# DerrickWang005/CRIS.pytorch

Measured on AMD Instinct MI355X. Metric: train-step samples/sec, CRIS-R50 416x416 bs=64; loss parity vs ref, higher is better.
Workload: dtype bf16; 1 GPU; CRIS-R50 bf16 training step (fwd+BCE+bwd+Adam), 416x416, per-GPU bs=8, 17-token text, synthetic RefCOCO-shape batch resident in HBM (BASELINE.json configs[1]); global_batch=8, parallelism=dp1, launch=graph, graph_captured=True, syncbn_exchange=none, grad_exchange=none

## Files before the change

cris/pytorch_amd/csrc/elementwise.hip:

```cpp
#include <cmath>
#include "common.h"
#include "../../../include/cris_hip.h"

__device__ __forceinline__ void ld8f(const float* p, float* f) {
    const float4 a = *reinterpret_cast<const float4*>(p);
    const float4 b = *reinterpret_cast<const float4*>(p + 4);
    f[0] = a.x; f[1] = a.y; f[2] = a.z; f[3] = a.w; f[4] = b.x; f[5] = b.y; f[6] = b.z; f[7] = b.w;
}
__device__ __forceinline__ void ld8bf(const bf16_t* p, float* f) { unpack8(*reinterpret_cast<const uint4*>(p), f); }
__device__ __forceinline__ void st8bf(bf16_t* p, const float* f) { *reinterpret_cast<uint4*>(p) = pack8(f); }

#define GRID_STRIDE(idx, total) \
    for (long idx = (long)blockIdx.x * blockDim.x + threadIdx.x; idx < (total); idx += (long)gridDim.x * blockDim.x)

__global__ void stem_im2col_kernel(const float* __restrict__ img, int Bn, int H, int W, int OH, int OW, bf16_t* __restrict__ out) {
    const long total = (long)Bn * OH * OW * 4;
    const bool small = total < (1L << 24);
    GRID_STRIDE(idx, total) {
        const cris_idx4 q = cris_split4(idx, 4, OW, OH, small);
        const int kc = q.cv, ow = q.x, oh = q.y, b = q.b;
        const long m = idx >> 2;
        float v[8];
#pragma unroll
        for (int j = 0; j < 8; ++j) {
            const int k = kc * 8 + j;
            float x = 0.f;
            if (k < 27) {
                const int ci = k / 9, t = k - ci * 9;
                const int kh = t / 3, kw = t - kh * 3;
                const int ih = oh * 2 + kh - 1, iw = ow * 2 + kw - 1;
                if ((unsigned)ih < (unsigned)H && (unsigned)iw < (unsigned)W) x = img[(((size_t)b * 3 + ci) * H + ih) * W + iw];
            }
            v[j] = x;
        }
        st8bf(out + m * 32 + kc * 8, v);
    }
}

extern "C" int cris_stem_im2col(const float* img, int Bn, int H, int W, cris_bf16* out, void* stream) {
    CRIS_CHECK_ARG(img && out && Bn > 0 && H > 0 && W > 0, "bad args");
    const int OH = (H + 2 - 3) / 2 + 1, OW = (W + 2 - 3) / 2 + 1;
    const long total = (long)Bn * OH * OW * 4;
    hipLaunchKernelGGL(stem_im2col_kernel, dim3(cris_grid_1d(total, 256)), dim3(256), 0, (hipStream_t)stream, img, Bn, H, W, OH, OW, out);
    CRIS_LAUNCH_CHECK();
    return 0;
}

__global__ void avgpool2_fwd_kernel(const bf16_t* __restrict__ x, int ldx, int xcoff, int Bn, int H, int W, int C,
                                    bf16_t* __restrict__ y, int ldy, int ycoff) {
    const int CV = C >> 3, OH = H >> 1, OW = W >> 1;
    const long total = (long)Bn * OH * OW * CV;
    const bool small = total < (1L << 24);
    GRID_STRIDE(idx, total) {
        const cris_idx4 q = cris_split4(idx, CV, OW, OH, small);
        const int cv = q.cv, ow = q.x, oh = q.y, b = q.b;
        const long mo = ((long)b * OH + oh) * OW + ow;
        float o[8] = {0, 0, 0, 0, 0, 0, 0, 0}, t[8];
#pragma unroll
        for (int dy = 0; dy < 2; ++dy)
#pragma unroll
            for (int dx = 0; dx < 2; ++dx) {
                ld8bf(x + (((size_t)b * H + oh * 2 + dy) * W + ow * 2 + dx) * ldx + xcoff + cv * 8, t);
#pragma unroll
                for (int j = 0; j < 8; ++j) o[j] += t[j];
            }
#pragma unroll
        for (int j = 0; j < 8; ++j) o[j] *= 0.25f;
        st8bf(y + (size_t)mo * ldy + ycoff + cv * 8, o);
    }
}

extern "C" int cris_avgpool2_fwd(const cris_bf16* x, int ldx, int xcoff, int Bn, int H, int W, int C, cris_bf16* y,
                                 int ldy, int ycoff, void* stream) {
    CRIS_CHECK_ARG(x && y && !(H & 1) && !(W & 1) && !(C & 7) && !(ldx & 7) && !(ldy & 7) && !(xcoff & 7) && !(ycoff & 7), "bad args");
    const long total = (long)Bn * (H / 2) * (W / 2) * (C / 8);
    hipLaunchKernelGGL(avgpool2_fwd_kernel, dim3(cris_grid_1d(total, 256)), dim3(256), 0, (hipStream_t)stream, x, ldx, xcoff,
                       Bn, H, W, C, y, ldy, ycoff);
    CRIS_LAUNCH_CHECK();
    return 0;
}

__global__ void avgpool2_bwd_kernel(const bf16_t* __restrict__ dy, int lddy, int dycoff, int Bn, int H, int W, int C,
                                    bf16_t* __restrict__ dx, int lddx, int dxcoff, int accum) {
    const int CV = C >> 3, OH = H >> 1, OW = W >> 1;
    const long total = (long)Bn * H * W * CV;
    const bool small = total < (1L << 24);
    GRID_STRIDE(idx, total) {
        const cris_idx4 q = cris_split4(idx, CV, W, H, small);
        const int cv = q.cv, w = q.x, h = q.y, b = q.b;
        const long m = ((long)b * H + h) * W + w;
        float g[8];
        ld8bf(dy + (((size_t)b * OH + (h >> 1)) * OW + (w >> 1)) * lddy + dycoff + cv * 8, g);
        bf16_t* d = dx + (size_t)m * lddx + dxcoff + cv * 8;
        float o[8];
        if (accum) ld8bf(d, o);
#pragma unroll
        for (int j = 0; j < 8; ++j) o[j] = (accum ? o[j] : 0.f) + 0.25f * g[j];
        st8bf(d, o);
    }
}

extern "C" int cris_avgpool2_bwd(const cris_bf16* dy, int lddy, int dycoff, int Bn, int H, int W, int C, cris_bf16* dx,
                                 int lddx, int dxcoff, int accum, void* stream) {
    CRIS_CHECK_ARG(dy && dx && !(H & 1) && !(W & 1) && !(C & 7) && !(lddx & 7) && !(lddy & 7) && !(dxcoff & 7) && !(dycoff & 7), "bad args");
    const long total = (long)Bn * H * W * (C / 8);
    hipLaunchKernelGGL(avgpool2_bwd_kernel, dim3(cris_grid_1d(total, 256)), dim3(256), 0, (hipStream_t)stream, dy, lddy, dycoff,
                       Bn, H, W, C, dx, lddx, dxcoff, accum);
    CRIS_LAUNCH_CHECK();
    return 0;
}

__device__ __forceinline__ void up2_src(int dst, int n_in, int& i0, int& i1, float& l1) {
    float s = (dst + 0.5f) * 0.5f - 0.5f;
    s = fmaxf(s, 0.f);
    i0 = (int)s;
    i1 = i0 < n_in - 1 ? i0 + 1 : i0;
    l1 = s - (float)i0;
}

__global__ void upsample2_fwd_kernel(const bf16_t* __restrict__ x, int ldx, int xcoff, int Bn, int H, int W, int C,
                                     bf16_t* __restrict__ y, int ldy, int ycoff) {
    const int CV = C >> 3, OH = H * 2, OW = W * 2;
    const long total = (long)Bn * OH * OW * CV;
    const bool small = total < (1L << 24);
    GRID_STRIDE(idx, total) {
        const cris_idx4 q = cris_split4(idx, CV, OW, OH, small);
        const int cv = q.cv, ow = q.x, oh = q.y, b = q.b;
        const long mo = ((long)b * OH + oh) * OW + ow;
        int y0, y1, x0, x1;
        float ly, lx;
        up2_src(oh, H, y0, y1, ly);
        up2_src(ow, W, x0, x1, lx);
        const bf16_t* base = x + (size_t)b * H * W * ldx + xcoff + cv * 8;
        float a[8], bb[8], c[8], d[8], o[8];
        ld8bf(base + ((size_t)y0 * W + x0) * ldx, a);
        ld8bf(base + ((size_t)y0 * W + x1) * ldx, bb);
        ld8bf(base + ((size_t)y1 * W + x0) * ldx, c);
        ld8bf(base + ((size_t)y1 * W + x1) * ldx, d);
        const float w00 = (1.f - ly) * (1.f - lx), w01 = (1.f - ly) * lx, w10 = ly * (1.f - lx), w11 = ly * lx;
#pragma unroll
        for (int j = 0; j < 8; ++j) o[j] = w00 * a[j] + w01 * bb[j] + w10 * c[j] + w11 * d[j];
        st8bf(y + (size_t)mo * ldy + ycoff + cv * 8, o);
    }
}

extern "C" int cris_upsample2_fwd(const cris_bf16* x, int ldx, int xcoff, int Bn, int H, int W, int C, cris_bf16* y,
                                  int ldy, int ycoff, void* stream) {
    CRIS_CHECK_ARG(x && y && !(C & 7) && !(ldx & 7) && !(ldy & 7) && !(xcoff & 7) && !(ycoff & 7), "bad args");
    const long total = (long)Bn * H * W * 4 * (C / 8);
    hipLaunchKernelGGL(upsample2_fwd_kernel, dim3(cris_grid_1d(total, 256)), dim3(256), 0, (hipStream_t)stream, x, ldx, xcoff,
                       Bn, H, W, C, y, ldy, ycoff);
    CRIS_LAUNCH_CHECK();
    return 0;
}

__global__ void upsample2_bwd_kernel(const bf16_t* __restrict__ dy, int lddy, int dycoff, int Bn, int H, int W, int C,
                                     bf16_t* __restrict__ dx, int lddx, int dxcoff, int accum) {
    const int CV = C >> 3, OH = H * 2, OW = W * 2;
    const long total = (long)Bn * H * W * CV;
    const bool small = total < (1L << 24);
    GRID_STRIDE(idx, total) {
        const cris_idx4 q = cris_split4(idx, CV, W, H, small);
        const int cv = q.cv, ix = q.x, iy = q.y, b = q.b;
        const long m = ((long)b * H + iy) * W + ix;
        float acc[8] = {0, 0, 0, 0, 0, 0, 0, 0};
        const bf16_t* base = dy + (size_t)b * OH * OW * lddy + dycoff + cv * 8;
        for (int oy = max(0, 2 * iy - 2); oy <= min(OH - 1, 2 * iy + 2); ++oy) {
            int y0, y1; float ly;
            up2_src(oy, H, y0, y1, ly);
            float wy = 0.f;
            if (y0 == iy) wy += 1.f - ly;
            if (y1 == iy) wy += ly;
            if (wy == 0.f) continue;
            for (int ox = max(0, 2 * ix - 2); ox <= min(OW - 1, 2 * ix + 2); ++ox) {
                int x0, x1; float lx;
                up2_src(ox, W, x0, x1, lx);
                float wx = 0.f;
                if (x0 == ix) wx += 1.f - lx;
                if (x1 == ix) wx += lx;
                if (wx == 0.f) continue;
                float g[8];
                ld8bf(base + ((size_t)oy * OW + ox) * lddy, g);
                const float w = wy * wx;
#pragma unroll
                for (int j = 0; j < 8; ++j) acc[j] += w * g[j];
            }
        }
        bf16_t* d = dx + (size_t)m * lddx + dxcoff + cv * 8;
        if (accum) {
            float o[8];
            ld8bf(d, o);
#pragma unroll
            for (int j = 0; j < 8; ++j) acc[j] += o[j];
        }
        st8bf(d, acc);
    }
}

extern "C" int cris_upsample2_bwd(const cris_bf16* dy, int lddy, int dycoff, int Bn, int H, int W, int C, cris_bf16* dx,
                                  int lddx, int dxcoff, int accum, void* stream) {
    CRIS_CHECK_ARG(dy && dx && !(C & 7) && !(lddx & 7) && !(lddy & 7) && !(dxcoff & 7) && !(dycoff & 7), "bad args");
    const long total = (long)Bn * H * W * (C / 8);
    hipLaunchKernelGGL(upsample2_bwd_kernel, dim3(cris_grid_1d(total, 256)), dim3(256), 0, (hipStream_t)stream, dy, lddy, dycoff,
                       Bn, H, W, C, dx, lddx, dxcoff, accum);
    CRIS_LAUNCH_CHECK();
    return 0;
}

__device__ __forceinline__ float linspace_m1_1(int i, int n) {
    if (n == 1) return -1.f;
    const float step = 2.f / (float)(n - 1);
    return i < n / 2 ? -1.f + step * (float)i : 1.f - step * (float)(n - 1 - i);
}

__global__ void fill_coords_kernel(bf16_t* x, int ldx, int coff, int nfill, int Bn, int H, int W) {
    const long total = (long)Bn * H * W;
    GRID_STRIDE(m, total) {
        const int w = (int)(m % W);
        const int h = (int)((m / W) % H);
        bf16_t* d = x + (size_t)m * ldx + coff;
        d[0] = f2bf(linspace_m1_1(w, W));
        d[1] = f2bf(linspace_m1_1(h, H));
        for (int j = 2; j < nfill; ++j) d[j] = 0;
    }
}

extern "C" int cris_fill_coords(cris_bf16* x, int ldx, int coff, int nfill, int Bn, int H, int W, void* stream) {
    CRIS_CHECK_ARG(x && nfill >= 2, "bad args");
    hipLaunchKernelGGL(fill_coords_kernel, dim3(cris_grid_1d((long)Bn * H * W, 256)), dim3(256), 0, (hipStream_t)stream, x, ldx,
                       coff, nfill, Bn, H, W);
    CRIS_LAUNCH_CHECK();
    return 0;
}

__global__ void gather_samples_kernel(const bf16_t* __restrict__ x, int ldx, int xcoff, const int32_t* __restrict__ index,
                                      int R, int CV, bf16_t* __restrict__ y, int ldy, int ycoff, int total) {
    for (int idx = blockIdx.x * blockDim.x + threadIdx.x; idx < total; idx += gridDim.x * blockDim.x) {
        const int cv = idx % CV;
        const int row = idx / CV;
        const int k = row / R;
        const int r = row - k * R;
        const long src = (long)index[k] * R + r;
        const uint4 v = *reinterpret_cast<const uint4*>(x + (size_t)src * ldx + xcoff + cv * 8);
        *reinterpret_cast<uint4*>(y + (size_t)row * ldy + ycoff + cv * 8) = v;
    }
}

extern "C" int cris_gather_samples_bf16(const cris_bf16* x, int ldx, int xcoff, const int32_t* index, int K,
                                        int rows_per_sample, int C, cris_bf16* y, int ldy, int ycoff, void* stream) {
    CRIS_CHECK_ARG(x && y && index && K > 0 && rows_per_sample > 0 && C > 0, "bad args");
    CRIS_CHECK_ARG(!(C & 7) && !(ldx & 7) && !(ldy & 7) && !(xcoff & 7) && !(ycoff & 7) && xcoff >= 0 && ycoff >= 0 &&
                   xcoff + C <= ldx && ycoff + C <= ldy, "channels, leading dimensions and offsets: multiples of 8, slice inside the row");
    CRIS_CHECK_ARG((long)K * rows_per_sample * ldy * 2 < (1L << 31), "output extent of 2 GiB or more");
    const int total = K * rows_per_sample * (C / 8);
    hipLaunchKernelGGL(gather_samples_kernel, dim3(cris_grid_1d(total, 256)), dim3(256), 0, (hipStream_t)stream, x, ldx, xcoff,
                       index, rows_per_sample, C / 8, y, ldy, ycoff, total);
    CRIS_LAUNCH_CHECK();
    return 0;
}

__global__ void add_bf16_kernel(const bf16_t* a, int lda, int acoff, const bf16_t* b, int ldb, int bcoff, bf16_t* y, int ldy,
                                int ycoff, int M, int C) {
    const int CV = C >> 3;
    const long total = (long)M * CV;
    GRID_STRIDE(idx, total) {
        const int cv = (int)(idx % CV);
        const long m = idx / CV;
        float u[8], v[8];
        ld8bf(a + (size_t)m * lda + acoff + cv * 8, u);
        if (b) {
            ld8bf(b + (size_t)m * ldb + bcoff + cv * 8, v);
#pragma unroll
            for (int j = 0; j < 8; ++j) u[j] += v[j];
        }
        st8bf(y + (size_t)m * ldy + ycoff + cv * 8, u);
    }
}

extern "C" int cris_add_bf16(const cris_bf16* a, int lda, int acoff, const cris_bf16* b, int ldb, int bcoff, cris_bf16* y,
                             int ldy, int ycoff, int M, int C, void* stream) {
    CRIS_CHECK_ARG(a && y && !(C & 7) && !(lda & 7) && !(ldy & 7) && !(acoff & 7) && !(ycoff & 7) && (!b || (!(ldb & 7) && !(bcoff & 7))), "bad args");
    hipLaunchKernelGGL(add_bf16_kernel, dim3(cris_grid_1d((long)M * (C / 8), 256)), dim3(256), 0, (hipStream_t)stream, a, lda,
                       acoff, b, ldb, bcoff, y, ldy, ycoff, M, C);
    CRIS_LAUNCH_CHECK();
    return 0;
}

__global__ void add_rowtable_kernel(const bf16_t* a, int lda, const float* table, int trows, bf16_t* y, int ldy, int M, int C) {
    const int CV = C >> 3;
    const long total = (long)M * CV;
    GRID_STRIDE(idx, total) {
        const int cv = (int)(idx % CV);
        const long m = idx / CV;
        float u[8], v[8];
        ld8bf(a + (size_t)m * lda + cv * 8, u);
        ld8f(table + (size_t)(m % trows) * C + cv * 8, v);
#pragma unroll
        for (int j = 0; j < 8; ++j) u[j] += v[j];
        st8bf(y + (size_t)m * ldy + cv * 8, u);
    }
}

extern "C" int cris_add_rowtable(const cris_bf16* a, int lda, const float* table, int trows, cris_bf16* y, int ldy, int M,
                                 int C, void* stream) {
    CRIS_CHECK_ARG(a && table && y && trows > 0 && !(C & 7) && !(lda & 7) && !(ldy & 7), "bad args");
    hipLaunchKernelGGL(add_rowtable_kernel, dim3(cris_grid_1d((long)M * (C / 8), 256)), dim3(256), 0, (hipStream_t)stream, a,
                       lda, table, trows, y, ldy, M, C);
    CRIS_LAUNCH_CHECK();
    return 0;
}

__global__ void cast_f32_bf16_kernel(const float* x, bf16_t* y, long n) {
    GRID_STRIDE(i, n) y[i] = f2bf(x[i]);
}
extern "C" int cris_cast_f32_bf16(const float* x, cris_bf16* y, long n, void* stream) {
    CRIS_CHECK_ARG(x && y && n > 0, "bad args");
    hipLaunchKernelGGL(cast_f32_bf16_kernel, dim3(cris_grid_1d(n, 256)), dim3(256), 0, (hipStream_t)stream, x, y, n);
    CRIS_LAUNCH_CHECK();
    return 0;
}
__global__ void cast_bf16_f32_kernel(const bf16_t* x, float* y, long n, int accum) {
    GRID_STRIDE(i, n) y[i] = (accum ? y[i] : 0.f) + bf2f(x[i]);
}
extern "C" int cris_cast_bf16_f32(const cris_bf16* x, float* y, long n, int accum, void* stream) {
    CRIS_CHECK_ARG(x && y && n > 0, "bad args");
    hipLaunchKernelGGL(cast_bf16_f32_kernel, dim3(cris_grid_1d(n, 256)), dim3(256), 0, (hipStream_t)stream, x, y, n, accum);
    CRIS_LAUNCH_CHECK();
    return 0;
}
__global__ void quickgelu_fwd_kernel(const bf16_t* x, bf16_t* y, long nvec) {
    GRID_STRIDE(i, nvec) {
        float v[8];
        ld8bf(x + i * 8, v);
#pragma unroll
        for (int j = 0; j < 8; ++j) v[j] = v[j] / (1.f + __expf(-1.702f * v[j]));
        st8bf(y + i * 8, v);
    }
}
extern "C" int cris_quickgelu_fwd(const cris_bf16* x, cris_bf16* y, long n, void* stream) {
    CRIS_CHECK_ARG(x && y && n > 0 && !(n & 7), "n must be a multiple of 8");
    hipLaunchKernelGGL(quickgelu_fwd_kernel, dim3(cris_grid_1d(n / 8, 256)), dim3(256), 0, (hipStream_t)stream, x, y, n / 8);
    CRIS_LAUNCH_CHECK();
    return 0;
}
__global__ void quickgelu_bwd_kernel(const bf16_t* x, const bf16_t* dy, bf16_t* dx, long nvec) {
    GRID_STRIDE(i, nvec) {
        float v[8], g[8];
        ld8bf(x + i * 8, v);
        ld8bf(dy + i * 8, g);
#pragma unroll
        for (int j = 0; j < 8; ++j) {
            const float s = 1.f / (1.f + __expf(-1.702f * v[j]));
            g[j] *= s * (1.f + 1.702f * v[j] * (1.f - s));
        }
        st8bf(dx + i * 8, g);
    }
}
extern "C" int cris_quickgelu_bwd(const cris_bf16* x, const cris_bf16* dy, cris_bf16* dx, long n, void* stream) {
    CRIS_CHECK_ARG(x && dy && dx && n > 0 && !(n & 7), "n must be a multiple of 8");
    hipLaunchKernelGGL(quickgelu_bwd_kernel, dim3(cris_grid_1d(n / 8, 256)), dim3(256), 0, (hipStream_t)stream, x, dy, dx, n / 8);
    CRIS_LAUNCH_CHECK();
    return 0;
}
__global__ void cast_drop_kernel(const float* x, bf16_t* y, long n, float scale, uint32_t thresh, uint32_t seed, uint32_t stream_id,
                                 const uint32_t* seed_dev) {
    const uint32_t key = cris_drop_key(seed + (seed_dev ? seed_dev[0] : 0u), stream_id);
    GRID_STRIDE(i, n) {
        float v = x[i];
        if (thresh) v = cris_keep(key, (uint32_t)i, thresh) ? v * scale : 0.f;
        y[i] = f2bf(v);
    }
}
extern "C" int cris_cast_f32_bf16_drop(const float* x, cris_bf16* y, long n, float drop_p, uint32_t drop_thresh, uint32_t seed,
                                       uint32_t stream_id, const uint32_t* seed_dev, void* stream) {
    CRIS_CHECK_ARG(x && y && n > 0 && n < (1L << 32), "bad args");
    const float scale = drop_thresh ? 1.f / (1.f - drop_p) : 1.f;
    hipLaunchKernelGGL(cast_drop_kernel, dim3(cris_grid_1d(n, 256)), dim3(256), 0, (hipStream_t)stream, x, y, n, scale, drop_thresh,
                       seed, stream_id, seed_dev);
    CRIS_LAUNCH_CHECK();
    return 0;
}
__global__ void step_advance_kernel(int* step, uint32_t* seed, int* exchange_gen) {
    const int s = step[0];
    seed[0] = (uint32_t)s * 7919u + 17u;
    step[0] = s + 1;
    if (exchange_gen) exchange_gen[0] += 1;
}
extern "C" int cris_step_advance(int32_t* step, uint32_t* seed, int32_t* exchange_gen, void* stream) {
    CRIS_CHECK_ARG(step && seed, "bad args");
    hipLaunchKernelGGL(step_advance_kernel, dim3(1), dim3(1), 0, (hipStream_t)stream, step, seed, exchange_gen);
    CRIS_LAUNCH_CHECK();
    return 0;
}
__global__ void step_advance_micro_kernel(int* step, uint32_t* seed, int* exchange_gen, int micro, int accum) {
    int s = step[0];
    if (micro == 0) step[0] = s + 1;
    else s -= 1;
    seed[0] = ((uint32_t)s * (uint32_t)accum + (uint32_t)micro) * 7919u + 17u;
    if (exchange_gen) exchange_gen[0] += 1;
}
extern "C" int cris_step_advance_micro(int32_t* step, uint32_t* seed, int32_t* exchange_gen, int micro, int accum, void* stream) {
    CRIS_CHECK_ARG(step && seed && accum >= 1 && micro >= 0 && micro < accum, "bad args (0 <= micro < accum)");
    hipLaunchKernelGGL(step_advance_micro_kernel, dim3(1), dim3(1), 0, (hipStream_t)stream, step, seed, exchange_gen, micro, accum);
    CRIS_LAUNCH_CHECK();
    return 0;
}
template <int MODE>
__global__ __launch_bounds__(256) void grad_accumulate_kernel(float4* __restrict__ dst, const float4* __restrict__ src, long nvec) {
    const long stride = (long)gridDim.x * 256;
    long i = (long)blockIdx.x * 256 + threadIdx.x;
    for (; i + stride < nvec; i += 2 * stride) {
        float4 s0 = src[i], s1 = src[i + stride];
        if (MODE == 1) {
            const float4 d0 = dst[i], d1 = dst[i + stride];
            s0.x = d0.x + s0.x; s0.y = d0.y + s0.y; s0.z = d0.z + s0.z; s0.w = d0.w + s0.w;
            s1.x = d1.x + s1.x; s1.y = d1.y + s1.y; s1.z = d1.z + s1.z; s1.w = d1.w + s1.w;
        }
        dst[i] = s0;
        dst[i + stride] = s1;
    }
    if (i < nvec) {
        float4 s0 = src[i];
        if (MODE == 1) {
            const float4 d0 = dst[i];
            s0.x = d0.x + s0.x; s0.y = d0.y + s0.y; s0.z = d0.z + s0.z; s0.w = d0.w + s0.w;
        }
        dst[i] = s0;
    }
}
static int cris_cu_count() {
    static int cached[64];
    int dev = 0;
    if (hipGetDevice(&dev) != hipSuccess || dev < 0 || dev >= 64) return 256;
    if (!cached[dev]) {
        int cus = 0;
        if (hipDeviceGetAttribute(&cus, hipDeviceAttributeMultiprocessorCount, dev) != hipSuccess || cus <= 0) cus = 256;
        cached[dev] = cus;
    }
    return cached[dev];
}
extern "C" int cris_grad_accumulate(float* dst, const float* src, long n, int mode, void* stream) {
    CRIS_CHECK_ARG(dst && src && n > 0 && !(n & 3), "n must be a positive multiple of 4");
    CRIS_CHECK_ARG(!(((uintptr_t)dst | (uintptr_t)src) & 15), "dst and src must be 16-byte aligned");
    CRIS_CHECK_ARG(mode == 0 || mode == 1, "mode must be 0 (dst = src) or 1 (dst += src)");
    CRIS_CHECK_ARG(dst + n <= src || src + n <= dst, "dst and src overlap");
    const long nvec = n >> 2;
    const int grid = cris_grid_1d(nvec, 512, 8 * cris_cu_count());
    if (mode == 0)
        hipLaunchKernelGGL(grad_accumulate_kernel<0>, dim3(grid), dim3(256), 0, (hipStream_t)stream, (float4*)dst, (const float4*)src, nvec);
    else
        hipLaunchKernelGGL(grad_accumulate_kernel<1>, dim3(grid), dim3(256), 0, (hipStream_t)stream, (float4*)dst, (const float4*)src, nvec);
    CRIS_LAUNCH_CHECK();
    return 0;
}
__global__ void axpy_f32_kernel(float* dst, const float* src, float alpha, long n) {
    GRID_STRIDE(i, n) dst[i] += alpha * src[i];
}
extern "C" int cris_axpy_f32(float* dst, const float* src, float alpha, long n, void* stream) {
    CRIS_CHECK_ARG(dst && src && n > 0, "bad args");
    hipLaunchKernelGGL(axpy_f32_kernel, dim3(cris_grid_1d(n, 256)), dim3(256), 0, (hipStream_t)stream, dst, src, alpha, n);
    CRIS_LAUNCH_CHECK();
    return 0;
}
__global__ void embed_fwd_kernel(const int64_t* tokens, const float* table, const float* pos, int Bn, int L, int D, float* out) {
    const int DV = D >> 2;
    const long total = (long)Bn * L * DV;
    GRID_STRIDE(idx, total) {
        const int dv = (int)(idx % DV);
        const long r = idx / DV;
        const int l = (int)(r % L);
        const int64_t tok = tokens[r];
        const float4 e = *reinterpret_cast<const float4*>(table + (size_t)tok * D + dv * 4);
        const float4 q = *reinterpret_cast<const float4*>(pos + (size_t)l * D + dv * 4);
        *reinterpret_cast<float4*>(out + (size_t)r * D + dv * 4) = make_float4(e.x + q.x, e.y + q.y, e.z + q.z, e.w + q.w);
    }
}
extern "C" int cris_embed_fwd(const int64_t* tokens, const float* table, const float* pos, int Bn, int L, int D, float* out,
                              void* stream) {
    CRIS_CHECK_ARG(tokens && table && pos && out && !(D & 3), "bad args");
    hipLaunchKernelGGL(embed_fwd_kernel, dim3(cris_grid_1d((long)Bn * L * (D / 4), 256)), dim3(256), 0, (hipStream_t)stream,
                       tokens, table, pos, Bn, L, D, out);
    CRIS_LAUNCH_CHECK();
    return 0;
}
__global__ void embed_bwd_kernel(const int64_t* tokens, const float* dx, int Bn, int L, int D, float* dtable, float* dpos,
                                 unsigned char* row_live) {
    const long total = (long)Bn * L * D;
    const int R = Bn * L;
    GRID_STRIDE(idx, total) {
        const int d = (int)(idx % D);
        const int r = (int)(idx / D);
        const int64_t tok = tokens[r];
        bool first = true;
        for (int q = 0; q < r; ++q) first = first && tokens[q] != tok;
        if (first) {
            float a = 0.f;
            for (int q = r; q < R; ++q)
                if (tokens[q] == tok) a += dx[(size_t)q * D + d];
            dtable[(size_t)tok * D + d] = a;
            if (row_live && d == 0) row_live[tok] = 1;
        }
        if (r < L) {
            float a = 0.f;
            for (int b = 0; b < Bn; ++b) a += dx[((size_t)b * L + r) * D + d];
            dpos[(size_t)r * D + d] = a;
// ... 812 lines not shown
```

cris/pytorch_amd/csrc/norm.hip:

```cpp
#include "common.h"
#include "../../../include/cris_hip.h"
#include "p2p_ll.h"
#include <string.h>

#define BN_WIDE_MIN 128
#define BN_MERGE_MIN 512
#define BN_MERGE_SLICES 64

template <int PL>
__device__ __forceinline__ float bn_lane_sum(float (*sh)[17], float v, int pl, int cl) {
    __syncthreads();
    sh[pl][cl] = v;
    __syncthreads();
    if (PL == 64) {
        float g = 0.f;
        if (pl < 8) {
#pragma unroll
            for (int j = 0; j < 8; ++j) g += sh[pl * 8 + j][cl];
        }
        __syncthreads();
        if (pl < 8) sh[pl][cl] = g;
        __syncthreads();
    }
    float t = sh[0][cl];
// ... 972 lines not shown
#pragma unroll
        for (int u = 0; u < U; ++u) {
            const int mu = m + u * step;
            if (mu >= M) break;
            float y[8], dz[8], z[8], g[8], o[8];
            unpack8(ry[u], y);
            unpack8(rdz[u], dz);
            if (MASK == 1) unpack8(rz[u], z);
#pragma unroll
            for (int j = 0; j < 8; ++j) {
                bool pos = true;
                if (MASK == 1) pos = z[j] > 0.f;
                if (MASK == 2) pos = (y[j] * sc[j] + sh[j]) > 0.f;
                g[j] = pos ? dz[j] : 0.f;
                const float xh = (y[j] - mean[j]) * inv[j];
                o[j] = sc[j] * (g[j] - a0[j] - xh * s1[j] * invc);
            }
            cris_st16(dyb + (size_t)mu * p.lddy, pack8(o));
            if (want2) {
                float y2[8];
                unpack8(ry2[u], y2);
#pragma unroll
                for (int j = 0; j < 8; ++j) {
                    const float xh2 = (y2[j] - mean2[j]) * inv2[j];
                    o[j] = sc2[j] * (g[j] - a0[j] - xh2 * s3[j] * invc);
                }
                cris_st16(dy2b + (size_t)mu * p.lddy2, pack8(o));
            }
            if (dib) {
                if (di_acc) {
                    float old[8];
                    unpack8(rold[u], old);
#pragma unroll
                    for (int j = 0; j < 8; ++j) g[j] += old[j];
                }
                cris_st16(dib + (size_t)mu * p.lddi, pack8(g));
            }
        }
    }
}

extern "C" int cris_bn_bwd_apply(const cris_bn_bwd_params* pp, void* stream) {
    const cris_bn_bwd_params& p = *pp;
    CRIS_CHECK_ARG(p.dz && p.y && p.mean && p.invstd && p.sums && p.scale && p.dy, "null operand");
    CRIS_CHECK_ARG((p.C & 7) == 0 && (p.lddy & 7) == 0 && (p.dy_coff & 7) == 0 && p.count > 0.f, "geometry");
    CRIS_CHECK_ARG(!(p.relu && !p.pool && p.y2 && !p.z), "relu over two branches takes its mask from the stored output z");
    const long total = (long)p.Bn * p.H * p.W * (p.C >> 3);
    static const int use_fast = cris_env_int("CRIS_BN_APPLY_FAST", 1);
    const int cvs = bn_cv_shift(p.C);
    const bool aligned = (p.ldy & 7) == 0 && (p.y_coff & 7) == 0 && (p.lddz & 7) == 0 && (p.dz_coff & 7) == 0 &&
                         (!p.y2 || ((p.ldy2 & 7) == 0 && (p.y2_coff & 7) == 0 && p.z && (!p.dy2 || ((p.lddy2 & 7) == 0 && (p.dy2_coff & 7) == 0)))) &&
                         (!p.dident || ((p.lddi & 7) == 0 && (p.di_coff & 7) == 0));
    if (use_fast && cvs >= 0 && !p.pool && !p.mul && aligned) {
        const int mask = !p.relu ? 0 : (p.y2 || p.z) ? 1 : 2;
        if (mask != 1 || ((p.ldz & 7) == 0 && (p.z_coff & 7) == 0)) {
            const int grid = bn_fast_grid(total, p.y2 ? 2 : 4);
            typedef void (*fn_t)(const cris_bn_bwd_params, int);
            static const fn_t tab[2][3] = {{bn_bwd_apply_fast_kernel<0, false>, bn_bwd_apply_fast_kernel<1, false>, bn_bwd_apply_fast_kernel<2, false>},
                                           {bn_bwd_apply_fast_kernel<0, true>, bn_bwd_apply_fast_kernel<1, true>, bn_bwd_apply_fast_kernel<2, true>}};
            hipLaunchKernelGGL(tab[p.y2 ? 1 : 0][mask], dim3(grid), dim3(256), 0, (hipStream_t)stream, p, cvs);
            CRIS_LAUNCH_CHECK();
            return 0;
        }
    }
    hipLaunchKernelGGL(bn_bwd_apply_kernel, dim3(cris_grid_1d(total, 256)), dim3(256), 0, (hipStream_t)stream, p);
    CRIS_LAUNCH_CHECK();
    return 0;
}

#define LN_MAXV 4

template <bool WANT_MASK, int V = LN_MAXV>
__device__ __forceinline__ void ln_load_row(const void* x, int x_f32, size_t rowoff, int C, int lane, int in_relu,
                                            uint32_t in_thresh, float in_scale, uint32_t in_key, uint32_t row,
                                            float (&v)[V][8], float (&mask_out)[V][8]) {
#pragma unroll
    for (int i = 0; i < V; ++i) {
        const int c0 = (lane + 64 * i) * 8;
        if (c0 < C) {
            if (x_f32) load8f(reinterpret_cast<const float*>(x) + rowoff + c0, v[i]);
            else load8bf(reinterpret_cast<const bf16_t*>(x) + rowoff + c0, v[i]);
#pragma unroll
            for (int j = 0; j < 8; ++j) {
                float m = 1.f;
                if (in_relu && !(v[i][j] > 0.f)) m = 0.f;
                if (in_thresh) m = cris_keep(in_key, row * (uint32_t)C + (uint32_t)(c0 + j), in_thresh) ? m * in_scale : 0.f;
                v[i][j] *= m;
                if (WANT_MASK) mask_out[i][j] = m;
            }
        } else {
#pragma unroll
            for (int j = 0; j < 8; ++j) {
                v[i][j] = 0.f;
                if (WANT_MASK) mask_out[i][j] = 0.f;
            }
        }
    }
}

__global__ __launch_bounds__(256) void ln_fwd_kernel(const cris_ln_fwd_params p) {
    const int lane = threadIdx.x & 63;
    const int wave_g = blockIdx.x * 4 + (threadIdx.x >> 6);
    const int nwaves = gridDim.x * 4;
    const uint32_t sdev = p.seed_dev ? p.seed_dev[0] : 0u;
    const uint32_t in_key = cris_drop_key(p.in_seed + sdev, p.in_stream);
    const uint32_t out_key = cris_drop_key(p.out_seed + sdev, p.out_stream);
    const float in_scale = p.in_thresh ? 1.f / (1.f - p.in_drop_p) : 1.f;
    const float out_scale = p.out_thresh ? 1.f / (1.f - p.out_drop_p) : 1.f;
    const float invC = 1.f / (float)p.C;
    for (int row = wave_g; row < p.rows; row += nwaves) {
        float v[LN_MAXV][8];
        ln_load_row<false>(p.x, p.x_f32, (size_t)row * p.ldx, p.C, lane, p.in_relu, p.in_thresh, in_scale, in_key, (uint32_t)row,
                           v, v);
        float s = 0.f;
#pragma unroll
        for (int i = 0; i < LN_MAXV; ++i)
#pragma unroll
            for (int j = 0; j < 8; ++j) s += v[i][j];
        const float mean = wave_sum(s) * invC;
        float q = 0.f;
#pragma unroll
        for (int i = 0; i < LN_MAXV; ++i) {
            const int c0 = (lane + 64 * i) * 8;
            if (c0 < p.C) {
#pragma unroll
                for (int j = 0; j < 8; ++j) {
                    const float d = v[i][j] - mean;
                    q += d * d;
                }
            }
        }
        const float rstd = rsqrtf(wave_sum(q) * invC + p.eps);
        if (lane == 0) {
            p.mean[row] = mean;
            p.rstd[row] = rstd;
        }
#pragma unroll
        for (int i = 0; i < LN_MAXV; ++i) {
            const int c0 = (lane + 64 * i) * 8;
            if (c0 >= p.C) continue;
            float ga[8], be[8], o[8];
            load8f(p.gamma + c0, ga);
            load8f(p.beta + c0, be);
#pragma unroll
            for (int j = 0; j < 8; ++j) o[j] = (v[i][j] - mean) * rstd * ga[j] + be[j];
            const size_t oo = (size_t)row * p.C + c0;
            if (p.y) cris_st16(p.y + oo, pack8(o));
            if (p.ypos) {
                float pe[8], t[8];
                load8f(p.pos + (size_t)(row % p.pos_rows) * p.C + c0, pe);
#pragma unroll
                for (int j = 0; j < 8; ++j) t[j] = o[j] + pe[j];
                cris_st16(p.ypos + oo, pack8(t));
            }
            if (p.out_f32) {
                float r[8];
                if (p.resid) load8f(p.resid + oo, r);
                else {
#pragma unroll
                    for (int j = 0; j < 8; ++j) r[j] = 0.f;
                }
#pragma unroll
                for (int j = 0; j < 8; ++j) {
                    float t = o[j];
                    if (p.out_thresh) t = cris_keep(out_key, (uint32_t)row * (uint32_t)p.C + (uint32_t)(c0 + j), p.out_thresh) ? t * out_scale : 0.f;
                    r[j] += t;
                }
                *reinterpret_cast<float4*>(p.out_f32 + oo) = make_float4(r[0], r[1], r[2], r[3]);
                *reinterpret_cast<float4*>(p.out_f32 + oo + 4) = make_float4(r[4], r[5], r[6], r[7]);
            }
        }
    }
}

extern "C" int cris_ln_fwd(const cris_ln_fwd_params* pp, void* stream) {
    const cris_ln_fwd_params& p = *pp;
    CRIS_CHECK_ARG(p.x && p.gamma && p.beta && p.mean && p.rstd && p.rows > 0, "null operand");
    CRIS_CHECK_ARG((p.C & 7) == 0 && p.C <= 64 * 8 * LN_MAXV && (p.ldx & 7) == 0, "C must be a multiple of 8, <= 2048");
    CRIS_CHECK_ARG(!p.ypos || (p.pos && p.pos_rows > 0), "ypos needs pos");
    CRIS_CHECK_ARG((long)p.rows * p.C < (1L << 32), "dropout index overflow");
    const int grid = cris_grid_1d(p.rows, 4, 2048);
    hipLaunchKernelGGL(ln_fwd_kernel, dim3(grid), dim3(256), 0, (hipStream_t)stream, p);
    CRIS_LAUNCH_CHECK();
    return 0;
}

template <int V>
__global__ __launch_bounds__(256) void ln_bwd_kernel(const cris_ln_bwd_params p) {
    __shared__ float sg[2][64 * 8 * V];
    const int lane = threadIdx.x & 63;
    const int wave_g = blockIdx.x * 4 + (threadIdx.x >> 6);
    const int nwaves = gridDim.x * 4;
    for (int i = threadIdx.x; i < 2 * 64 * 8 * V; i += 256) (&sg[0][0])[i] = 0.f;
    __syncthreads();
    const uint32_t sdev = p.seed_dev ? p.seed_dev[0] : 0u;
    const uint32_t in_key = cris_drop_key(p.in_seed + sdev, p.in_stream);
    const uint32_t out_key = cris_drop_key(p.out_seed + sdev, p.out_stream);
    const float in_scale = p.in_thresh ? 1.f / (1.f - p.in_drop_p) : 1.f;
    const float out_scale = p.out_thresh ? 1.f / (1.f - p.out_drop_p) : 1.f;
    const float invC = 1.f / (float)p.C;
    float dga[V][8], dbe[V][8];
#pragma unroll
    for (int i = 0; i < V; ++i)
#pragma unroll
        for (int j = 0; j < 8; ++j) dga[i][j] = dbe[i][j] = 0.f;

    for (int row = wave_g; row < p.rows; row += nwaves) {
        float v[V][8], msk[V][8];
        ln_load_row<true, V>(p.x, p.x_f32, (size_t)row * p.ldx, p.C, lane, p.in_relu, p.in_thresh, in_scale, in_key, (uint32_t)row,
                          v, msk);
        const float mean = p.mean[row], rstd = p.rstd[row];
        float a[V][8];
        float s1 = 0.f, s2 = 0.f;
#pragma unroll
        for (int i = 0; i < V; ++i) {
            const int c0 = (lane + 64 * i) * 8;
            if (c0 < p.C) {
                const size_t oo = (size_t)row * p.C + c0;
                float g[8], t[8], ga[8];
#pragma unroll
                for (int j = 0; j < 8; ++j) g[j] = 0.f;
                if (p.dy) {
                    load8bf(p.dy + oo, t);
#pragma unroll
                    for (int j = 0; j < 8; ++j) g[j] += t[j];
                }
                if (p.dypos) {
                    load8bf(p.dypos + oo, t);
#pragma unroll
                    for (int j = 0; j < 8; ++j) g[j] += t[j];
                }
                if (p.dout_f32) {
                    load8f(p.dout_f32 + oo, t);
#pragma unroll
                    for (int j = 0; j < 8; ++j) {
                        float d = t[j];
                        if (p.out_thresh) d = cris_keep(out_key, (uint32_t)row * (uint32_t)p.C + (uint32_t)(c0 + j), p.out_thresh) ? d * out_scale : 0.f;
                        g[j] += d;
                    }
                }
                load8f(p.gamma + c0, ga);
#pragma unroll
                for (int j = 0; j < 8; ++j) {
                    const float xh = (v[i][j] - mean) * rstd;
                    v[i][j] = xh;
                    dga[i][j] += g[j] * xh;
                    dbe[i][j] += g[j];
                    a[i][j] = g[j] * ga[j];
                    s1 += a[i][j];
                    s2 += a[i][j] * xh;
                }
            } else {
#pragma unroll
                for (int j = 0; j < 8; ++j) a[i][j] = 0.f;
            }
        }
        const float m1 = wave_sum(s1) * invC, m2 = wave_sum(s2) * invC;
#pragma unroll
        for (int i = 0; i < V; ++i) {
            const int c0 = (lane + 64 * i) * 8;
            if (c0 >= p.C) continue;
            float o[8];
#pragma unroll
            for (int j = 0; j < 8; ++j) o[j] = rstd * (a[i][j] - m1 - v[i][j] * m2) * msk[i][j];
            const size_t xo = (size_t)row * p.ldx + c0;
            if (p.dx_f32) {
                float* d = reinterpret_cast<float*>(p.dx) + xo;
                if (p.dx_accum) {
                    float old[8];
                    load8f(d, old);
#pragma unroll
                    for (int j = 0; j < 8; ++j) o[j] += old[j];
                }
                *reinterpret_cast<float4*>(d) = make_float4(o[0], o[1], o[2], o[3]);
                *reinterpret_cast<float4*>(d + 4) = make_float4(o[4], o[5], o[6], o[7]);
            } else {
                cris_st16(reinterpret_cast<bf16_t*>(p.dx) + xo, pack8(o));
            }
        }
    }
    for (int w = 0; w < 4; ++w) {
        if ((int)(threadIdx.x >> 6) == w) {
#pragma unroll
            for (int i = 0; i < V; ++i) {
                const int c0 = (lane + 64 * i) * 8;
                if (c0 < p.C) {
#pragma unroll
                    for (int j = 0; j < 8; ++j) {
                        sg[0][c0 + j] += dga[i][j];
                        sg[1][c0 + j] += dbe[i][j];
                    }
                }
            }
        }
        __syncthreads();
    }
    float* part = p.part + (size_t)blockIdx.x * 2 * p.C;
    for (int c = threadIdx.x; c < p.C; c += 256) {
        part[c] = sg[0][c];
        part[p.C + c] = sg[1][c];
    }
}

static int ln_bwd_grid(int rows) {
    static const int max_grid = cris_env_int("CRIS_LN_BWD_BLOCKS", 512);
    return cris_grid_1d(rows, 4, max_grid);
}
extern "C" int cris_ln_bwd_parts(int rows) { return ln_bwd_grid(rows); }

extern "C" int cris_ln_bwd(const cris_ln_bwd_params* pp, void* stream) {
    const cris_ln_bwd_params& p = *pp;
    CRIS_CHECK_ARG(p.x && p.gamma && p.mean && p.rstd && p.dx && p.part && p.rows > 0, "null operand");
    CRIS_CHECK_ARG(p.dy || p.dypos || p.dout_f32, "no incoming gradient");
    CRIS_CHECK_ARG((p.C & 7) == 0 && p.C <= 64 * 8 * LN_MAXV && (p.ldx & 7) == 0, "C must be a multiple of 8, <= 2048");
    CRIS_CHECK_ARG(!p.dx_accum || p.dx_f32, "accumulate only into fp32");
    static const int narrow = cris_env_int("CRIS_LN_BWD_V", 1);
    const dim3 grid(ln_bwd_grid(p.rows));
    if (narrow && p.C <= 512) hipLaunchKernelGGL(ln_bwd_kernel<1>, grid, dim3(256), 0, (hipStream_t)stream, p);
    else if (narrow && p.C <= 1024) hipLaunchKernelGGL(ln_bwd_kernel<2>, grid, dim3(256), 0, (hipStream_t)stream, p);
    else hipLaunchKernelGGL(ln_bwd_kernel<LN_MAXV>, grid, dim3(256), 0, (hipStream_t)stream, p);
    CRIS_LAUNCH_CHECK();
    return 0;
}

__global__ __launch_bounds__(256) void sum_group_kernel(const cris_sum_group g) {
    __shared__ float sh[4][64];
    int ei = 0;
#pragma unroll
    for (int i = 1; i < CRIS_SUM_GROUP_MAX; ++i) ei += g.block_start[i] <= (int)blockIdx.x ? 1 : 0;
    const cris_sum_entry e = g.e[ei];
    const int cl = threadIdx.x & 63, pl = threadIdx.x >> 6;
    const int c = (blockIdx.x - g.block_start[ei]) * 64 + cl;
    float a = 0.f;
    if (c < e.ncol)
        for (int i = pl; i < e.nparts; i += 4) a += e.part[(size_t)i * e.ld + c];
    sh[pl][cl] = a;
    __syncthreads();
    if (pl == 0 && c < e.ncol) e.out[c] = (sh[0][cl] + sh[1][cl]) + (sh[2][cl] + sh[3][cl]);
}

extern "C" int cris_sum_tables(const cris_sum_group* gp, void* stream) {
    CRIS_CHECK_ARG(gp && gp->n > 0 && gp->n <= CRIS_SUM_GROUP_MAX, "1 .. CRIS_SUM_GROUP_MAX tables per launch");
    cris_sum_group g = *gp;
    int start = 0;
    for (int i = 0; i < g.n; ++i) {
        CRIS_CHECK_ARG(g.e[i].part && g.e[i].out && g.e[i].nparts > 0 && g.e[i].ncol > 0 && g.e[i].ld >= g.e[i].ncol, "bad table");
        g.block_start[i] = start;
        start += cris_cdiv(g.e[i].ncol, 64);
    }
    for (int i = g.n; i <= CRIS_SUM_GROUP_MAX; ++i) g.block_start[i] = start;
    hipLaunchKernelGGL(sum_group_kernel, dim3(start), dim3(256), 0, (hipStream_t)stream, g);
    CRIS_LAUNCH_CHECK();
    return 0;
}
```

Measured before the change: 671.3 samples/s.

## Add quad-output upsample2 fwd, gather bwd, lean wide LN bwd, prefetching sum_tables

Adds an upsample2 forward kernel in which each thread loads a 3x3 input neighbourhood once and writes four output pixels, replacing four separate threads that each reloaded four neighbours. It also adds a backward kernel that enumerates exactly the four output rows and columns touching each input pixel, with fixed bilinear weights. A new LayerNorm backward kernel for C>1024 prefetches the next row's x and dy into registers and recomputes masks from bits to save registers. The partial-table sum kernel batches 16 independent loads per thread to expose memory-level parallelism. All four paths are on by default behind env flags. The code trades extra register pressure and a hardcoded half-pixel weight pattern for fewer redundant loads.

```diff
diff --git a/cris/pytorch_amd/csrc/elementwise.hip b/cris/pytorch_amd/csrc/elementwise.hip
--- a/cris/pytorch_amd/csrc/elementwise.hip
+++ b/cris/pytorch_amd/csrc/elementwise.hip
@@ -144,9 +144,62 @@
     }
 }
 
+__device__ __forceinline__ void up2_blend(const uint4 ra, const uint4 rb, const uint4 rc, const uint4 rd, float ly, float lx, bf16_t* dst) {
+    float a[8], bb[8], c[8], d[8], o[8];
+    unpack8(ra, a);
+    unpack8(rb, bb);
+    unpack8(rc, c);
+    unpack8(rd, d);
+    const float w00 = (1.f - ly) * (1.f - lx), w01 = (1.f - ly) * lx, w10 = ly * (1.f - lx), w11 = ly * lx;
+#pragma unroll
+    for (int j = 0; j < 8; ++j) o[j] = w00 * a[j] + w01 * bb[j] + w10 * c[j] + w11 * d[j];
+    st8bf(dst, o);
+}
+__device__ __forceinline__ uint4 up2_sel(bool first, const uint4 a, const uint4 b) {
+    return make_uint4(first ? a.x : b.x, first ? a.y : b.y, first ? a.z : b.z, first ? a.w : b.w);
+}
+
+__global__ void upsample2_fwd_quad_kernel(const bf16_t* __restrict__ x, int ldx, int xcoff, int Bn, int H, int W, int C,
+                                          bf16_t* __restrict__ y, int ldy, int ycoff) {
+    const int CV = C >> 3, OW = W * 2;
+    const long total = (long)Bn * H * W * CV;
+    const bool small = total < (1L << 24);
+    GRID_STRIDE(idx, total) {
+        const cris_idx4 q = cris_split4(idx, CV, W, H, small);
+        const int cv = q.cv, ix = q.x, iy = q.y, b = q.b;
+        int r[3], c[3], y1e, x1e;
+        float lye, lyo, lxe, lxo;
+        up2_src(2 * iy, H, r[0], y1e, lye);
+        up2_src(2 * iy + 1, H, r[1], r[2], lyo);
+        up2_src(2 * ix, W, c[0], x1e, lxe);
+        up2_src(2 * ix + 1, W, c[1], c[2], lxo);
+        const bf16_t* base = x + (size_t)b * H * W * ldx + xcoff + cv * 8;
+        uint4 v[3][3];
+#pragma unroll
+        for (int a = 0; a < 3; ++a)
+#pragma unroll
+            for (int e = 0; e < 3; ++e) v[a][e] = *reinterpret_cast<const uint4*>(base + ((size_t)r[a] * W + c[e]) * ldx);
+        const bool ym = y1e == r[1], xm = x1e == c[1];
+        uint4 t[3];
+#pragma unroll
+        for (int e = 0; e < 3; ++e) t[e] = up2_sel(ym, v[1][e], v[2][e]);
+        bf16_t* d = y + (((size_t)b * 2 * H + 2 * iy) * OW + 2 * ix) * ldy + ycoff + cv * 8;
+        up2_blend(v[0][0], up2_sel(xm, v[0][1], v[0][2]), t[0], up2_sel(xm, t[1], t[2]), lye, lxe, d);
+        up2_blend(v[0][1], v[0][2], t[1], t[2], lye, lxo, d + ldy);
+        up2_blend(v[1][0], up2_sel(xm, v[1][1], v[1][2]), v[2][0], up2_sel(xm, v[2][1], v[2][2]), lyo, lxe, d + (size_t)OW * ldy);
+        up2_blend(v[1][1], v[1][2], v[2][1], v[2][2], lyo, lxo, d + (size_t)OW * ldy + ldy);
+    }
+}
+
 extern "C" int cris_upsample2_fwd(const cris_bf16* x, int ldx, int xcoff, int Bn, int H, int W, int C, cris_bf16* y,
                                   int ldy, int ycoff, void* stream) {
     CRIS_CHECK_ARG(x && y && !(C & 7) && !(ldx & 7) && !(ldy & 7) && !(xcoff & 7) && !(ycoff & 7), "bad args");
+    if (cris_env_int("CRIS_UPSAMPLE2_QUAD", 1)) {
+        hipLaunchKernelGGL(upsample2_fwd_quad_kernel, dim3(cris_grid_1d((long)Bn * H * W * (C / 8), 256)), dim3(256), 0, (hipStream_t)stream,
+                           x, ldx, xcoff, Bn, H, W, C, y, ldy, ycoff);
+        CRIS_LAUNCH_CHECK();
+        return 0;
+    }
     const long total = (long)Bn * H * W * 4 * (C / 8);
     hipLaunchKernelGGL(upsample2_fwd_kernel, dim3(cris_grid_1d(total, 256)), dim3(256), 0, (hipStream_t)stream, x, ldx, xcoff,
                        Bn, H, W, C, y, ldy, ycoff);
@@ -197,10 +250,69 @@
     }
 }
 
+__device__ __forceinline__ void up2_hits(int i, int n, int on, int (&o)[4], float (&w)[4], bool (&ok)[4]) {
+    o[0] = max(2 * i - 1, 0);      w[0] = 0.25f;                      ok[0] = i >= 1;
+    o[1] = 2 * i;                  w[1] = i >= 1 ? 0.75f : 1.f;       ok[1] = true;
+    o[2] = 2 * i + 1;              w[2] = i == n - 1 ? 1.f : 0.75f;   ok[2] = true;
+    o[3] = min(2 * i + 2, on - 1); w[3] = 0.25f;                      ok[3] = i < n - 1;
+}
+
+__global__ void upsample2_bwd_enum_kernel(const bf16_t* __restrict__ dy, int lddy, int dycoff, int Bn, int H, int W, int C,
+                                          bf16_t* __restrict__ dx, int lddx, int dxcoff, int accum) {
+    const int CV = C >> 3, OH = H * 2, OW = W * 2;
+    const long total = (long)Bn * H * W * CV;
+    const bool small = total < (1L << 24);
+    GRID_STRIDE(idx, total) {
+        const cris_idx4 q = cris_split4(idx, CV, W, H, small);
+        const int cv = q.cv, ix = q.x, iy = q.y, b = q.b;
+        const long m = ((long)b * H + iy) * W + ix;
+        int oy[4], ox[4];
+        float wy[4], wx[4];
+        bool oky[4], okx[4];
+        up2_hits(iy, H, OH, oy, wy, oky);
+        up2_hits(ix, W, OW, ox, wx, okx);
+        const bf16_t* base = dy + (size_t)b * OH * OW * lddy + dycoff + cv * 8;
+        uint4 r[4][4];
+#pragma unroll
+        for (int a = 0; a < 4; ++a)
+#pragma unroll
+            for (int e = 0; e < 4; ++e) r[a][e] = *reinterpret_cast<const uint4*>(base + ((size_t)oy[a] * OW + ox[e]) * lddy);
+        bf16_t* d = dx + (size_t)m * lddx + dxcoff + cv * 8;
+        uint4 old = make_uint4(0, 0, 0, 0);
+        if (accum) old = *reinterpret_cast<const uint4*>(d);
+        float acc[8] = {0, 0, 0, 0, 0, 0, 0, 0};
+#pragma unroll
+        for (int a = 0; a < 4; ++a)
+#pragma unroll
+            for (int e = 0; e < 4; ++e) {
+                if (oky[a] && okx[e]) {
+                    float g[8];
+                    unpack8(r[a][e], g);
+                    const float w = wy[a] * wx[e];
+#pragma unroll
+                    for (int j = 0; j < 8; ++j) acc[j] += w * g[j];
+                }
+            }
+        if (accum) {
+            float o[8];
+            unpack8(old, o);
+#pragma unroll
+            for (int j = 0; j < 8; ++j) acc[j] += o[j];
+        }
+        st8bf(d, acc);
+    }
+}
+
 extern "C" int cris_upsample2_bwd(const cris_bf16* dy, int lddy, int dycoff, int Bn, int H, int W, int C, cris_bf16* dx,
                                   int lddx, int dxcoff, int accum, void* stream) {
     CRIS_CHECK_ARG(dy && dx && !(C & 7) && !(lddx & 7) && !(lddy & 7) && !(dxcoff & 7) && !(dycoff & 7), "bad args");
     const long total = (long)Bn * H * W * (C / 8);
+    if (cris_env_int("CRIS_UPSAMPLE2_QUAD", 1)) {
+        hipLaunchKernelGGL(upsample2_bwd_enum_kernel, dim3(cris_grid_1d(total, 256)), dim3(256), 0, (hipStream_t)stream, dy, lddy, dycoff,
+                           Bn, H, W, C, dx, lddx, dxcoff, accum);
+        CRIS_LAUNCH_CHECK();
+        return 0;
+    }
     hipLaunchKernelGGL(upsample2_bwd_kernel, dim3(cris_grid_1d(total, 256)), dim3(256), 0, (hipStream_t)stream, dy, lddy, dycoff,
                        Bn, H, W, C, dx, lddx, dxcoff, accum);
     CRIS_LAUNCH_CHECK();
diff --git a/cris/pytorch_amd/csrc/norm.hip b/cris/pytorch_amd/csrc/norm.hip
--- a/cris/pytorch_amd/csrc/norm.hip
+++ b/cris/pytorch_amd/csrc/norm.hip
@@ -1298,6 +1298,179 @@
     }
 }
 
+__device__ __forceinline__ uint32_t ln_lean_xh(const uint4 xr, int in_relu, uint32_t in_thresh, float in_scale, uint32_t in_key,
+                                               uint32_t idx0, float mean, float rstd, float* xh) {
+#pragma clang fp contract(off)
+    float v[8];
+    unpack8(xr, v);
+    uint32_t bits = 0;
+#pragma unroll
+    for (int j = 0; j < 8; ++j) {
+        float m = 1.f;
+        if (in_relu && !(v[j] > 0.f)) m = 0.f;
+        if (in_thresh) m = cris_keep(in_key, idx0 + (uint32_t)j, in_thresh) ? m * in_scale : 0.f;
+        v[j] *= m;
+        bits |= m != 0.f ? 1u << j : 0u;
+        xh[j] = (v[j] - mean) * rstd;
+    }
+    return bits;
+}
+__device__ __forceinline__ void ln_lean_xh_again(const uint4 xr, uint32_t bits, float mval, float mean, float rstd, float* xh, float* msk) {
+#pragma clang fp contract(off)
+    float v[8];
+    unpack8(xr, v);
+#pragma unroll
+    for (int j = 0; j < 8; ++j) {
+        const float m = (bits >> j) & 1u ? mval : 0.f;
+        v[j] *= m;
+        msk[j] = m;
+        xh[j] = (v[j] - mean) * rstd;
+    }
+}
+
+__device__ __forceinline__ void ln_lean_load(const cris_ln_bwd_params& p, const bf16_t* xb, int row, int lane, uint4 (&xr)[LN_MAXV],
+                                             uint4 (&dyr)[LN_MAXV], float& mean, float& rstd) {
+    const bf16_t* dyb = p.dy ? p.dy : xb;
+    const size_t xo = (size_t)row * p.ldx, dyo = p.dy ? (size_t)row * p.C : xo;
+#pragma unroll
+    for (int i = 0; i < LN_MAXV; ++i) {
+        const int c0 = (lane + 64 * i) * 8, cc = c0 < p.C ? c0 : 0;
+        xr[i] = *reinterpret_cast<const uint4*>(xb + xo + cc);
+        dyr[i] = *reinterpret_cast<const uint4*>(dyb + dyo + cc);
+    }
+    mean = p.mean[row];
+    rstd = p.rstd[row];
+}
+
+__global__ __launch_bounds__(256) void ln_bwd_lean_kernel(const cris_ln_bwd_params p) {
+    constexpr int V = LN_MAXV;
+    __shared__ float sg[2][64 * 8 * V];
+    __shared__ float sgam[64 * 8 * V];
+    const int lane = threadIdx.x & 63;
+    const int wave_g = blockIdx.x * 4 + (threadIdx.x >> 6);
+    const int nwaves = gridDim.x * 4;
+    for (int i = threadIdx.x; i < 2 * 64 * 8 * V; i += 256) (&sg[0][0])[i] = 0.f;
+    for (int i = threadIdx.x; i < p.C; i += 256) sgam[i] = p.gamma[i];
+    __syncthreads();
+    const uint32_t sdev = p.seed_dev ? p.seed_dev[0] : 0u;
+    const uint32_t in_key = cris_drop_key(p.in_seed + sdev, p.in_stream);
+    const uint32_t out_key = cris_drop_key(p.out_seed + sdev, p.out_stream);
+    const float in_scale = p.in_thresh ? 1.f / (1.f - p.in_drop_p) : 1.f;
+    const float out_scale = p.out_thresh ? 1.f / (1.f - p.out_drop_p) : 1.f;
+    const float invC = 1.f / (float)p.C;
+    const float mval = p.in_thresh ? 1.f * in_scale : 1.f;
+    const bf16_t* xb = reinterpret_cast<const bf16_t*>(p.x);
+    float dga[V][8], dbe[V][8];
+#pragma unroll
+    for (int i = 0; i < V; ++i)
+#pragma unroll
+        for (int j = 0; j < 8; ++j) dga[i][j] = dbe[i][j] = 0.f;
+
+    uint4 xr[V], dyr[V], xn[V], dyn[V];
+    float mean, rstd, mean_n, rstd_n;
+    ln_lean_load(p, xb, min(wave_g, p.rows - 1), lane, xr, dyr, mean, rstd);
+    for (int row = wave_g; row < p.rows; row += nwaves) {
+        ln_lean_load(p, xb, min(row + nwaves, p.rows - 1), lane, xn, dyn, mean_n, rstd_n);
+        float a[V][8];
+        float s1 = 0.f, s2 = 0.f;
+        uint32_t mbits = 0;
+#pragma unroll
+        for (int i = 0; i < V; ++i) {
+            const int c0 = (lane + 64 * i) * 8;
+            if (c0 < p.C) {
+                const size_t oo = (size_t)row * p.C + c0;
+                float g[8], t[8], ga[8], xh[8];
+#pragma unroll
+                for (int j = 0; j < 8; ++j) g[j] = 0.f;
+                if (p.dy) {
+                    unpack8(dyr[i], t);
+#pragma unroll
+                    for (int j = 0; j < 8; ++j) g[j] += t[j];
+                }
+                if (p.dypos) {
+                    load8bf(p.dypos + oo, t);
+#pragma unroll
+                    for (int j = 0; j < 8; ++j) g[j] += t[j];
+                }
+                if (p.dout_f32) {
+                    load8f(p.dout_f32 + oo, t);
+#pragma unroll
+                    for (int j = 0; j < 8; ++j) {
+                        float d = t[j];
+                        if (p.out_thresh) d = cris_keep(out_key, (uint32_t)row * (uint32_t)p.C + (uint32_t)(c0 + j), p.out_thresh) ? d * out_scale : 0.f;
+                        g[j] += d;
+                    }
+                }
+                load8f(sgam + c0, ga);
+                mbits |= ln_lean_xh(xr[i], p.in_relu, p.in_thresh, in_scale, in_key, (uint32_t)row * (uint32_t)p.C + (uint32_t)c0, mean, rstd, xh) << (8 * i);
+#pragma unroll
+                for (int j = 0; j < 8; ++j) {
+                    dga[i][j] += g[j] * xh[j];
+                    dbe[i][j] += g[j];
+                    a[i][j] = g[j] * ga[j];
+                    s1 += a[i][j];
+                    s2 += a[i][j] * xh[j];
+                }
+            } else {
+#pragma unroll
+                for (int j = 0; j < 8; ++j) a[i][j] = 0.f;
+            }
+        }
+        const float m1 = wave_sum(s1) * invC, m2 = wave_sum(s2) * invC;
+#pragma unroll
+        for (int i = 0; i < V; ++i) {
+            const int c0 = (lane + 64 * i) * 8;
+            if (c0 >= p.C) continue;
+            float o[8], xh[8], msk[8];
+            ln_lean_xh_again(xr[i], mbits >> (8 * i), mval, mean, rstd, xh, msk);
+#pragma unroll
+            for (int j = 0; j < 8; ++j) o[j] = rstd * (a[i][j] - m1 - xh[j] * m2) * msk[j];
+            const size_t xo = (size_t)row * p.ldx + c0;
+            if (p.dx_f32) {
+                float* d = reinterpret_cast<float*>(p.dx) + xo;
+                if (p.dx_accum) {
+                    float old[8];
+                    load8f(d, old);
+#pragma unroll
+                    for (int j = 0; j < 8; ++j) o[j] += old[j];
+                }
+                *reinterpret_cast<float4*>(d) = make_float4(o[0], o[1], o[2], o[3]);
+                *reinterpret_cast<float4*>(d + 4) = make_float4(o[4], o[5], o[6], o[7]);
+            } else {
+                cris_st16(reinterpret_cast<bf16_t*>(p.dx) + xo, pack8(o));
+            }
+        }
+#pragma unroll
+        for (int i = 0; i < V; ++i) {
+            xr[i] = xn[i];
+            dyr[i] = dyn[i];
+        }
+        mean = mean_n;
+        rstd = rstd_n;
+    }
+    for (int w = 0; w < 4; ++w) {
+        if ((int)(threadIdx.x >> 6) == w) {
+#pragma unroll
+            for (int i = 0; i < V; ++i) {
+                const int c0 = (lane + 64 * i) * 8;
+                if (c0 < p.C) {
+#pragma unroll
+                    for (int j = 0; j < 8; ++j) {
+                        sg[0][c0 + j] += dga[i][j];
+                        sg[1][c0 + j] += dbe[i][j];
+                    }
+                }
+            }
+        }
+        __syncthreads();
+    }
+    float* part = p.part + (size_t)blockIdx.x * 2 * p.C;
+    for (int c = threadIdx.x; c < p.C; c += 256) {
+        part[c] = sg[0][c];
+        part[p.C + c] = sg[1][c];
+    }
+}
+
 static int ln_bwd_grid(int rows) {
     static const int max_grid = cris_env_int("CRIS_LN_BWD_BLOCKS", 512);
     return cris_grid_1d(rows, 4, max_grid);
@@ -1314,11 +1487,14 @@
     const dim3 grid(ln_bwd_grid(p.rows));
     if (narrow && p.C <= 512) hipLaunchKernelGGL(ln_bwd_kernel<1>, grid, dim3(256), 0, (hipStream_t)stream, p);
     else if (narrow && p.C <= 1024) hipLaunchKernelGGL(ln_bwd_kernel<2>, grid, dim3(256), 0, (hipStream_t)stream, p);
+    else if (p.C > 1024 && !p.x_f32 && cris_env_int("CRIS_LN_BWD_LEAN", 1)) hipLaunchKernelGGL(ln_bwd_lean_kernel, grid, dim3(256), 0, (hipStream_t)stream, p);
     else hipLaunchKernelGGL(ln_bwd_kernel<LN_MAXV>, grid, dim3(256), 0, (hipStream_t)stream, p);
     CRIS_LAUNCH_CHECK();
     return 0;
 }
 
+#define SUM_GROUP_AHEAD 16
+template <bool AHEAD>
 __global__ __launch_bounds__(256) void sum_group_kernel(const cris_sum_group g) {
     __shared__ float sh[4][64];
     int ei = 0;
@@ -1328,8 +1504,19 @@
     const int cl = threadIdx.x & 63, pl = threadIdx.x >> 6;
     const int c = (blockIdx.x - g.block_start[ei]) * 64 + cl;
     float a = 0.f;
-    if (c < e.ncol)
-        for (int i = pl; i < e.nparts; i += 4) a += e.part[(size_t)i * e.ld + c];
+    if (c < e.ncol) {
+        int i = pl;
+        if (AHEAD) {
+            for (; i + 4 * (SUM_GROUP_AHEAD - 1) < e.nparts; i += 4 * SUM_GROUP_AHEAD) {
+                float v[SUM_GROUP_AHEAD];
+#pragma unroll
+                for (int k = 0; k < SUM_GROUP_AHEAD; ++k) v[k] = e.part[(size_t)(i + 4 * k) * e.ld + c];
+#pragma unroll
+                for (int k = 0; k < SUM_GROUP_AHEAD; ++k) a += v[k];
+            }
+        }
+        for (; i < e.nparts; i += 4) a += e.part[(size_t)i * e.ld + c];
+    }
     sh[pl][cl] = a;
     __syncthreads();
     if (pl == 0 && c < e.ncol) e.out[c] = (sh[0][cl] + sh[1][cl]) + (sh[2][cl] + sh[3][cl]);
@@ -1345,7 +1532,8 @@
         start += cris_cdiv(g.e[i].ncol, 64);
     }
     for (int i = g.n; i <= CRIS_SUM_GROUP_MAX; ++i) g.block_start[i] = start;
-    hipLaunchKernelGGL(sum_group_kernel, dim3(start), dim3(256), 0, (hipStream_t)stream, g);
+    if (cris_env_int("CRIS_SUM_GROUP_AHEAD", 1)) hipLaunchKernelGGL(sum_group_kernel<true>, dim3(start), dim3(256), 0, (hipStream_t)stream, g);
+    else hipLaunchKernelGGL(sum_group_kernel<false>, dim3(start), dim3(256), 0, (hipStream_t)stream, g);
     CRIS_LAUNCH_CHECK();
     return 0;
 }
```

Measured after the change: 674.7 samples/s, median of 6. About the same (+0.5%).
